# catniplab/vlgp

Hardware: AMD Instinct MI355X
Metric: EM iterations/sec (higher is better)
Workload: dtype f64

## Files before the change

vlgp_amd/csrc/ctx.h:

```cpp
#pragma once
#include <hip/hip_runtime.h>
#include <stdint.h>

#include <map>
#include <string>
#include <vector>

#include "../../include/vlgp_hip.h"

#define VLGP_WAVE 64
#define VLGP_E_LANES 4
#define VLGP_PRIOR_SLOTS 64

struct Prior {
    int T = 0;
    double* d_full = nullptr;
    double* d_compact = nullptr;
    std::vector<int> rl;
    std::vector<int64_t> goff;
    int64_t compact_len = 0;
    int index = -1;
};

enum : unsigned {
    SET_PLAIN = 1,
    SET_TILING = 2,
    SET_COPIED = 4,
    SET_GROUPS = 8,
    SET_MASKED = 16,
    SET_MASKED_FIT = 32,
    SET_REPLICATED = SET_GROUPS | SET_MASKED | SET_MASKED_FIT,
    SET_BY_ROW = SET_MASKED | SET_MASKED_FIT,
    SET_FIT = SET_PLAIN | SET_TILING | SET_COPIED | SET_MASKED_FIT,
    SET_SOURCE = 64,
    SET_ANY = 127,
};

struct Replicas {
    int src = -1;
    bool by_row = false, overlap = false;
    int n = 0, n_pairs = 0, nw = 0;
    int64_t rows_src = 0;
    int* d_ch = nullptr;
    int* d_pair = nullptr;
    unsigned long long* d_mask = nullptr;
    double* d_wconst = nullptr;
    double* d_nobs = nullptr;
    void* d_xa = nullptr;
    double xh[8] = {};
};

struct UnitSet {
    bool valid = false;
    int M = 0;
    int64_t rows = 0;
    int Tmax = 0, Tmin = 0;
    std::vector<int64_t> off;
    int64_t* d_off = nullptr;
    double *y = nullptr, *x = nullptr, *mu = nullptr, *v = nullptr, *w = nullptr, *dmu = nullptr;
    bool x_ones = true;
    bool alias = false;
    int parent = -1;
    std::vector<int64_t> src_start;
    int64_t* d_src_start = nullptr;
    int* d_unit_prior = nullptr;
    uint64_t prior_epoch = 0;
    double* d_xb = nullptr;
    double* d_mu_stash = nullptr;
    double* d_scratch = nullptr;
    int64_t scratch_len = 0;
    double rows_all_ranks = 0.0;
    std::vector<int> stage_start;
    std::vector<int> link_start;
    int* d_links = nullptr;
    int n_links = 0;
    bool share_mu = true;
    Replicas rep;
    int rep_users = 0;

    unsigned kind() const {
        if (rep.src >= 0) return !rep.by_row ? SET_GROUPS : (rep.n == 1 ? SET_MASKED_FIT : SET_MASKED);
        return alias ? SET_TILING : (parent >= 0 ? SET_COPIED : SET_PLAIN);
    }
    bool is(unsigned kinds) const { return (kind() & kinds) != 0; }
    bool is_source() const { return rep_users > 0; }
};

#define VLGP_SWITCHES(X)                                                                                                 \
    X("VLGP_ESTEP_SPLIT", estep_split, TRI, -1, 0, 1, "split E-step (chip-wide launches per phase): 0 never, 1 whatever the set's size") \
    X("VLGP_ESTEP_LSPLIT", estep_lsplit, TRI, -1, 0, 1, "long units (T > 64) on the split E-step: 0 never, 1 below 128 tasks too") \
    X("VLGP_ESTEP_GENERIC", estep_generic, FLAG, false, 0, 1, "E-step: the generic kernels only (a replicated set keeps the split E-step)") \
    X("VLGP_ESTEP_LANEPT", estep_lanept, TRI, -1, 0, 1, "split E-step: 0 keeps the wave-per-task kernels for ranks <= 14") \
    X("VLGP_ESTEP_NO_SHARED_G", estep_no_shared_g, FLAG, false, 0, 1, "split E-step: per-wave staging of G in the rank <= 16 launches, no lane-per-task launches") \
    X("VLGP_ESTEP_MIX", estep_mix, TRI, -1, 0, 1, "split E-step: 0 launches lane-per-task and wave-per-task latents separately") \
    X("VLGP_ESTEP_LANES", estep_lanes, INT, 0, 1, VLGP_E_LANES, "split E-step: number of stream lanes (default: by set size, one or two)") \
    X("VLGP_LANE_PRIO", lane_prio, INT, 0, 0, 3, "instruction priority of the lane-per-task launches' waves")                \
    X("VLGP_LANE_CLOCK", lane_clock, INT, 0, 0, 2, "phase clock of the lane-per-task launches: 1 factor, 2 mean (vlgp_debug_phase_clock)") \
    X("VLGP_MSTEP_GENERIC", mstep_generic, FLAG, false, 0, 1, "M-step: the loop-based kernels at any size")                    \
    X("VLGP_MSTEP_WG_PER_CU", mstep_wg_per_cu, REAL, 1.0, 0.0, 1e300, "M-step accumulation: workgroups per compute unit")       \
    X("VLGP_NOISE_PASSES", noise_passes, FLAG, false, 0, 1, "M-step: the noise variance by two passes over the rows, not from the moments") \
    X("VLGP_NO_MGRAPH", no_mgraph, FLAG, false, 0, 1, "M-step: enqueue every launch instead of replaying the captured graph") \
    X("VLGP_ICHOL_BLOCK", ichol_block, FLAG, false, 0, 1, "prior factor: lengths <= 64 through the workgroup kernel of the long ones") \
    X("VLGP_NORMS_BLOCKS", norms_blocks, INT, 256, 1, 1024, "norms pass: largest number of workgroups (its partial sums have 1024 slots)") \
    X("VLGP_HSTEP_DENSE", hstep_dense, FLAG, false, 0, 1, "H-step: the dense matrix-pipe round, never the low-rank one")     \
    X("VLGP_HSTEP_GENERIC", hstep_generic, FLAG, false, 0, 1, "H-step: the generic kernels (the reference's omega retry)")     \
    X("VLGP_HSTEP_LOWRANK", hstep_lowrank, FLAG, false, 0, 1, "H-step: the low-rank round whatever the size rule says")        \
    X("VLGP_HSTEP_GENERIC_SEG", hstep_generic_seg, FLAG, false, 0, 1, "H-step: windows 65 ... 128 on the generic kernels")     \
    X("VLGP_HSTEP_FUSE_TABLES", hstep_fuse_tables, FLAG, false, 0, 1, "H-step: every low-rank round workgroup factors its kernel blocks itself (rejected: slower)") \
    X("VLGP_HSTEP_NO_WLM", hstep_no_wlm, FLAG, false, 0, 1, "H-step: the rounds read w row-major, no latent-major copy")       \
    X("VLGP_HSTEP_LR_TOL", hstep_lr_tol, REAL, 1e-12, 0.0, 1e300, "H-step: relative tolerance of the low-rank round's rank prediction") \
    X("VLGP_DEBUG_OCC", debug_occ, FLAG, false, 0, 1, "print occupancy of the fast E-step launch and the H-step's fall-backs on stderr")
#define VLGP_SW_T_FLAG bool
#define VLGP_SW_T_TRI int
#define VLGP_SW_T_INT int
#define VLGP_SW_T_REAL double
struct Switches {
#define X(name, field, kind, def, lo, hi, what) VLGP_SW_T_##kind field = def;
    VLGP_SWITCHES(X)
#undef X
};
void vlgp_read_switches(struct vlgp_ctx* ctx);

struct ProfSlot {
    int64_t launches = 0;
    double ms = 0.0;
    double units = 0.0;
};

struct vlgp_ctx {
    int dev = 0;
    hipStream_t stream = nullptr;
    int N = 0, L = 0, P = 0, R = 0;
    int n_cu = 256;
    std::vector<uint8_t> gauss;
    int n_gauss = 0;
    int* d_gauss = nullptr;
    double *d_a = nullptr, *d_b = nullptr, *d_noise = nullptr, *d_da = nullptr, *d_db = nullptr;
    bool have_params = false;

    std::map<int, Prior> priors;
    uint64_t prior_epoch = 1;
    const double** d_prior_base = nullptr;
    int* d_prior_rl = nullptr;
    int64_t* d_prior_goff = nullptr;
    int prior_rows = 0;
    int* h_prior_mb = nullptr;
    int* d_prior_mb_host = nullptr;
    int* d_prior_mb = nullptr;
    unsigned long long prior_seq = 0;
    std::vector<struct Prior*> prior_pending;
    unsigned long long prior_pending_seq = 0;

    UnitSet sets[VLGP_MAX_SETS];

    hipStream_t mstream = nullptr;
    double* d_work_m = nullptr;
    int64_t work_m_len = 0;
    int* d_fail_m = nullptr;
    void* comm_m = nullptr;
    hipEvent_t ev_fork = nullptr, ev_m_start = nullptr, ev_m_done = nullptr;
    bool m_pending = false;
    void* m_graph_exec = nullptr;
    std::vector<double> m_graph_key;

    double* d_ecols = nullptr;
    int* d_fail = nullptr;
    unsigned long long* d_clk = nullptr;
    double* d_work = nullptr;
    int64_t work_len = 0;
    double* h_pinned = nullptr;
    int64_t pinned_len = 0;
    unsigned* d_hsync = nullptr;
    double* h_hres = nullptr;
    double* d_hres = nullptr;
    unsigned h_seq = 0;
    double* d_hmpart = nullptr;
    bool hprep = false;
    hipEvent_t ev_e_done = nullptr;
    bool e_done_valid = false;
    uint64_t hprep_epoch = 0, write_epoch = 0;
    double* d_hmom = nullptr;
    int64_t hmom_len = 0;
    const UnitSet* hmom_us = nullptr;
    int hmom_T = 0;
    bool hmom_bracket = false;
    double* d_hwlm = nullptr;
    int64_t hwlm_len = 0;
    bool hwlm_valid = false;
    struct LrThr { int T; double dt, tol; std::vector<double> om; };
    std::vector<LrThr> lr_thr;
    Switches sw;
    std::vector<const void*> lds_attr_done;
    int h_prio = 1;
    double last_h_ms = 0.0, last_m_ms = 0.0;
    double h_t0 = 0.0;
    int last_hstep_path = 0;
    double hstat[4] = {0.0, 0.0, 0.0, 0.0};

    bool prof_on = false;
    ProfSlot prof[VLGP_PROF_KINDS];
    hipEvent_t ev0 = nullptr, ev1 = nullptr;
    struct PendingProf { int kind; hipEvent_t a, b; double units; bool done; };
    std::vector<PendingProf> pending;

    void* comm = nullptr;
    void* shm = nullptr;
    void* shm_m = nullptr;
    void* hx = nullptr;
    int rank = 0, world = 1;

    hipStream_t elane[VLGP_E_LANES - 1] = {};
    hipEvent_t ev_e_fork = nullptr, ev_e_join[VLGP_E_LANES - 1] = {};
    int last_estep_path = 0;
    int lds_max = 64 * 1024;

    double* d_xwork = nullptr;
    double* h_xres = nullptr;
    double* d_xres = nullptr;
    unsigned long long x_seq = 0;
    int x_pending = 0;
    int x_set = -1;
    double* h_msnap = nullptr;
    double* d_msnap = nullptr;
    bool msnap_valid = false;
    double* h_stage_par = nullptr;
    double* h_stage_map = nullptr;
    double* d_stage_map = nullptr;
    hipEvent_t ev_stage_par = nullptr, ev_stage_map = nullptr;
    bool stage_par_busy = false, stage_map_busy = false;

    double* d_elbo = nullptr;
    int64_t elbo_len = 0;

    std::string err;
};

inline UnitSet& vlgp_rows_owner(vlgp_ctx* ctx, UnitSet& us) { return us.rep.src >= 0 ? ctx->sets[us.rep.src] : us; }

struct LoglikShape { int64_t slots, n_rate; int grid_y; const char* limit; };
inline LoglikShape vlgp_loglik_shape(const vlgp_ctx* ctx, const UnitSet& us) {
    if (us.is(SET_BY_ROW))
        return {(int64_t)us.rep.n * ctx->N, us.rep.rows_src * ctx->N, us.rep.n, "vlgp_loglik: at most 65535 replicas per masked set"};
    if (us.is(SET_GROUPS))
        return {us.rep.n_pairs, us.rep.rows_src * us.rep.n_pairs, us.rep.n_pairs,
                "vlgp_loglik: at most 65535 (replica, channel) pairs per set"};
    return {ctx->N, us.rows * ctx->N, 1, ""};
}

int vlgp_fail(vlgp_ctx* ctx, int code, const char* fmt, ...);
#define HIPCHK(ctx, call)                                                          \
    do {                                                                           \
        hipError_t e__ = (call);                                                   \
// ... 71 lines not shown
```

vlgp_amd/csrc/mstep.hip:

```cpp
#include <type_traits>

#include "ctx.h"
#include "fast_exp.h"

#ifndef M_TILE
#define M_TILE 256
#endif

enum { K_PREP = 0, K_NEWTON = 1, K_NOISE1 = 2, K_NOISE2 = 3 };
enum { K_MASKED = 4 };

struct MArgs {
    int N, L, P;
    int64_t rows;
    int rows_per_wg;
    int CT;
    int S;
    const double* y;
    const double* x;
    const double* mu;
    const double* v;
    const double* a;
    const double* b;
    union {
        const int* gauss;
        const unsigned long long* mask;
    };
    union {
        const double* mean;
        const double* nobs;
    };
    double* partial;
};

__host__ __device__ constexpr int tri(int n) { return n * (n + 1) / 2; }
template <int LT, int PT, int KINDM>
__host__ __device__ constexpr int nacc() {
    constexpr int KIND = KINDM & (K_MASKED - 1);
    return KIND == K_PREP ? LT + PT + PT * LT + tri(PT) + (PT <= 2 ? 2 + PT : 0)
         : KIND == K_NEWTON ? 2 * LT + tri(LT) + PT + tri(PT)
         : 1;
}
static inline int nstat_rt(int L, int P, int kind) {
    return kind == K_PREP ? L + P + P * L + tri(P) + (P <= 2 ? 2 + P : 0) : kind == K_NEWTON ? 2 * L + tri(L) + P + tri(P) : 1;
}

#define MS_GS 8
template <int LT, int PT, int KINDM, bool EXACT>
__global__ void __launch_bounds__(512, (LT <= 5 ? 4 : (LT <= 8 ? 2 : 1))) mstep_accum(MArgs A) {
    extern __shared__ __attribute__((aligned(16))) double smem[];
    constexpr int KIND = KINDM & (K_MASKED - 1);
    constexpr bool MASKED = (KINDM & K_MASKED) != 0;
    constexpr int NA = nacc<LT, PT, KIND>();
    constexpr int NBUF = 1;
    const int N = A.N, CT = A.CT, S = A.S;
    const int L = EXACT ? LT : A.L, P = EXACT ? PT : A.P;
    const int tid = threadIdx.x;
    const int nl = tid % CT, s = tid / CT;
    const int n = blockIdx.y * CT + nl;
    const bool active = s < S && n < N;
    const int tile_d = 2 * M_TILE * L;
    double* red = smem;
    const int red_d = MS_GS * S * CT;
    double* etab = smem + (NBUF * tile_d > red_d ? NBUF * tile_d : red_d);
    if constexpr (KIND == K_NEWTON) fast_exp_tab_init(etab, tid);

    double al[LT], al2[LT], bl[PT], acc[NA];
#pragma unroll
    for (int l = 0; l < LT; ++l) {
        al[l] = (active && l < L) ? A.a[l * N + n] : 0.0;
        al2[l] = 0.5 * al[l] * al[l];
    }
#pragma unroll
    for (int j = 0; j < PT; ++j) bl[j] = (active && j < P) ? A.b[j * N + n] : 0.0;
#pragma unroll
    for (int k = 0; k < NA; ++k) acc[k] = 0.0;
    const bool gch = (active && !MASKED) ? A.gauss[n] != 0 : false;
    const int nw = (N + 63) >> 6;
    if constexpr (MASKED && KIND == K_NEWTON) {
        if (active && s == 0 && blockIdx.x == 0 && A.nobs[n] == 0.0) {
#pragma unroll
            for (int i = 0; i < LT; ++i) acc[LT + tri(i) + i] = 1.0;
#pragma unroll
            for (int i = 0; i < PT; ++i) acc[2 * LT + tri(LT) + PT + tri(i) + i] = 1.0;
        }
    }
    const double shift = (KIND == K_NOISE2 && active) ? A.mean[n] : 0.0;

    const int64_t c0 = (int64_t)blockIdx.x * A.rows_per_wg;
    int64_t c1 = c0 + A.rows_per_wg;
    if (c1 > A.rows) c1 = A.rows;
    auto copy_tile = [&](double* buf, int64_t t0) {
        const int cnt = (int)((c1 - t0) < M_TILE ? (c1 - t0) : M_TILE) * L;
        for (int i = tid; i < cnt; i += blockDim.x) {
            buf[i] = A.mu[t0 * L + i];
            buf[M_TILE * L + i] = A.v[t0 * L + i];
        }
    };
    if (c0 < c1) copy_tile(smem, c0);
    __syncthreads();
    for (int64_t t0 = c0; t0 < c1; t0 += M_TILE) {
        const int nr = (int)((c1 - t0) < M_TILE ? (c1 - t0) : M_TILE);
        const bool more = t0 + M_TILE < c1;
        const double* mu_t = smem;
        const double* v_t = mu_t + M_TILE * L;
        if (active && !(KIND == K_NEWTON && gch)) {
#pragma unroll 2
        for (int rr = s; rr < nr; rr += S) {
            const int64_t row = t0 + rr;
            double xv[PT];
#pragma unroll
            for (int j = 0; j < PT; ++j)
                xv[j] = EXACT ? 1.0 : ((j < P) ? (A.x ? A.x[(row * P + j) * N + n] : 1.0) : 0.0);
            double mr[LT], vr[LT];
#pragma unroll
            for (int l = 0; l < LT; ++l) {
                mr[l] = (EXACT || l < L) ? mu_t[rr * L + l] : 0.0;
                vr[l] = (EXACT || l < L) ? v_t[rr * L + l] : 0.0;
            }
            auto observed = [&]() -> bool {
                return ((reinterpret_cast<const unsigned*>(A.mask)[row * (2 * nw) + (n >> 5)] >> (n & 31)) & 1u) == 0u;
            };
            if constexpr (KIND == K_PREP) {
                double yv = A.y[row * N + n];
                if constexpr (MASKED) yv = observed() ? yv : 0.0;
                int k = 0;
#pragma unroll
                for (int l = 0; l < LT; ++l) { acc[k] = fma(mr[l], yv, acc[k]); ++k; }
#pragma unroll
                for (int j = 0; j < PT; ++j) { acc[k] = fma(xv[j], yv, acc[k]); ++k; }
#pragma unroll
                for (int j = 0; j < PT; ++j)
#pragma unroll
                    for (int l = 0; l < LT; ++l) { acc[k] = fma(xv[j], mr[l], acc[k]); ++k; }
#pragma unroll
                for (int i = 0; i < PT; ++i)
#pragma unroll
                    for (int j = 0; j <= i; ++j) { acc[k] = fma(xv[i], xv[j], acc[k]); ++k; }
                if constexpr (PT <= 2) {
                    acc[k] = fma(yv, yv, acc[k]); ++k;
                    acc[k] += yv; ++k;
#pragma unroll
                    for (int j = 0; j < PT; ++j) { acc[k] += xv[j]; ++k; }
                }
            } else {
                double eta = 0.0;
#pragma unroll
                for (int j = 0; j < PT; ++j) eta = fma(xv[j], bl[j], eta);
#pragma unroll
                for (int l = 0; l < LT; ++l) eta = fma(mr[l], al[l], eta);
                if constexpr (KIND == K_NEWTON) {
                    double ex = eta;
#pragma unroll
                    for (int l = 0; l < LT; ++l) ex = fma(vr[l], al2[l], ex);
                    double rate = trunc_exp_tab64(ex, etab);
                    if constexpr (MASKED) rate = observed() ? rate : 0.0;
                    double mt[LT], q[LT];
#pragma unroll
                    for (int l = 0; l < LT; ++l) {
                        mt[l] = fma(vr[l], al[l], mr[l]);
                        q[l] = mt[l] * rate;
                    }
                    int k = 0;
#pragma unroll
                    for (int l = 0; l < LT; ++l) { acc[k] += q[l]; ++k; }
#pragma unroll
                    for (int i = 0; i < LT; ++i)
#pragma unroll
                        for (int j = 0; j <= i; ++j) { acc[k] = fma(q[i], mt[j], acc[k]); ++k; }
#pragma unroll
                    for (int l = 0; l < LT; ++l) { acc[k] = fma(rate, vr[l], acc[k]); ++k; }
#pragma unroll
                    for (int j = 0; j < PT; ++j) { acc[k] = fma(xv[j], rate, acc[k]); ++k; }
#pragma unroll
                    for (int i = 0; i < PT; ++i)
#pragma unroll
                        for (int j = 0; j <= i; ++j) { acc[k] = fma(xv[i] * xv[j], rate, acc[k]); ++k; }
                } else {
                    double dres = A.y[row * N + n] - eta - shift;
                    if constexpr (MASKED) dres = observed() ? dres : 0.0;
                    if constexpr (KIND == K_NOISE1) acc[0] += dres;
                    else acc[0] = fma(dres, dres, acc[0]);
                }
            }
        }
        }
        if (more) {
            __syncthreads();
            copy_tile(smem, t0 + M_TILE);
        }
        __syncthreads();
    }
    int kex[NA];
    {
        int k = 0, ke = 0;
        if constexpr (KIND == K_PREP) {
#pragma unroll
            for (int l = 0; l < LT; ++l, ++k) kex[k] = l < L ? ke++ : -1;
#pragma unroll
            for (int j = 0; j < PT; ++j, ++k) kex[k] = j < P ? ke++ : -1;
#pragma unroll
            for (int j = 0; j < PT; ++j)
#pragma unroll
                for (int l = 0; l < LT; ++l, ++k) kex[k] = (j < P && l < L) ? ke++ : -1;
#pragma unroll
            for (int i = 0; i < PT; ++i)
#pragma unroll
                for (int j = 0; j <= i; ++j, ++k) kex[k] = i < P ? ke++ : -1;
            if constexpr (PT <= 2) {
                kex[k++] = ke++;
                kex[k++] = ke++;
#pragma unroll
                for (int j = 0; j < PT; ++j, ++k) kex[k] = j < P ? ke++ : -1;
            }
        } else if constexpr (KIND == K_NEWTON) {
#pragma unroll
            for (int l = 0; l < LT; ++l, ++k) kex[k] = l < L ? ke++ : -1;
#pragma unroll
            for (int i = 0; i < LT; ++i)
#pragma unroll
                for (int j = 0; j <= i; ++j, ++k) kex[k] = i < L ? ke++ : -1;
#pragma unroll
            for (int l = 0; l < LT; ++l, ++k) kex[k] = l < L ? ke++ : -1;
#pragma unroll
            for (int j = 0; j < PT; ++j, ++k) kex[k] = j < P ? ke++ : -1;
#pragma unroll
            for (int i = 0; i < PT; ++i)
#pragma unroll
                for (int j = 0; j <= i; ++j, ++k) kex[k] = i < P ? ke++ : -1;
        } else {
            kex[0] = 0;
        }
    }
    const int K = KIND == K_PREP ? L + P + P * L + tri(P) + (P <= 2 ? 2 + P : 0) : KIND == K_NEWTON ? 2 * L + tri(L) + P + tri(P) : 1;
    const int SC = S * CT;
#pragma unroll
    for (int g0 = 0; g0 < NA; g0 += MS_GS) {
        if (s < S) {
#pragma unroll
            for (int j = 0; j < MS_GS; ++j)
                if (g0 + j < NA) red[j * SC + s * CT + nl] = active ? acc[g0 + j] : 0.0;
        }
        __syncthreads();
        for (int o = tid; o < MS_GS * CT; o += blockDim.x) {
            const int j = o / CT, c = o - j * CT;
            int ke = -1;
#pragma unroll
            for (int jj = 0; jj < MS_GS; ++jj)
                if (g0 + jj < NA && jj == j) ke = kex[g0 + jj];
            const int nn = blockIdx.y * CT + c;
            if (ke >= 0 && nn < N) {
                double t = 0.0;
                for (int q = 0; q < S; ++q) t += red[j * SC + q * CT + c];
                A.partial[((int64_t)blockIdx.x * K + ke) * N + nn] = t;
            }
        }
        if (g0 + MS_GS < NA) __syncthreads();
    }
}

__global__ void __launch_bounds__(512) sum_partials_kernel(const double* partial, int G, int64_t K, double* out) {
    __shared__ double red[8][64];
    const int o = threadIdx.x & 63, sl = threadIdx.x >> 6;
    const int64_t i = (int64_t)blockIdx.x * 64 + o;
    double s0 = 0.0, s1 = 0.0;
    if (i < K) {
        int g = sl;
        for (; g + 8 < G; g += 16) {
            s0 += partial[(int64_t)g * K + i];
            s1 += partial[(int64_t)(g + 8) * K + i];
        }
        if (g < G) s0 += partial[(int64_t)g * K + i];
    }
    red[sl][o] = s0 + s1;
    __syncthreads();
    if (sl == 0 && i < K) {
        double t = 0.0;
#pragma unroll
        for (int q = 0; q < 8; ++q) t += red[q][o];
        out[i] = t;
    }
}

template <int LT>
__global__ void __launch_bounds__(256)
latent_moments_kernel(int L, int64_t rows, const double* mu, const double* v, const double* dmu,
                      double* partial) {
    __shared__ double red[256];
    constexpr int NA = tri(LT) + 3 * LT + 1;
    double acc[NA];
#pragma unroll
    for (int k = 0; k < NA; ++k) acc[k] = 0.0;
    for (int64_t t = (int64_t)blockIdx.x * 256 + threadIdx.x; t < rows; t += (int64_t)gridDim.x * 256) {
        double mr[LT], vr[LT], dr[LT];
#pragma unroll
        for (int l = 0; l < LT; ++l) {
            mr[l] = l < L ? mu[t * L + l] : 0.0;
            vr[l] = (v && l < L) ? v[t * L + l] : 0.0;
            dr[l] = (dmu && l < L) ? dmu[t * L + l] : 0.0;
        }
        int k = 0;
#pragma unroll
        for (int i = 0; i < LT; ++i)
#pragma unroll
            for (int j = 0; j <= i; ++j) { acc[k] = fma(mr[i], mr[j], acc[k]); ++k; }
#pragma unroll
        for (int l = 0; l < LT; ++l) { acc[k] += mr[l]; ++k; }
#pragma unroll
        for (int l = 0; l < LT; ++l) { acc[k] += vr[l]; ++k; }
#pragma unroll
        for (int l = 0; l < LT; ++l) { acc[k] = fma(mr[l], mr[l], acc[k]); ++k; }
#pragma unroll
        for (int l = 0; l < LT; ++l) acc[k] = fma(dr[l], dr[l], acc[k]);
    }
    const int K = tri(L) + 3 * L + 1;
    auto emit = [&](int ke, double val) {
        __syncthreads();
        red[threadIdx.x] = val;
        __syncthreads();
        for (int o = 128; o > 0; o >>= 1) {
            if ((int)threadIdx.x < o) red[threadIdx.x] += red[threadIdx.x + o];
            __syncthreads();
        }
        if (threadIdx.x == 0) partial[(int64_t)blockIdx.x * K + ke] = red[0];
    };
    int k = 0, ke = 0;
#pragma unroll
    for (int i = 0; i < LT; ++i)
#pragma unroll
        for (int j = 0; j <= i; ++j, ++k) if (i < L) emit(ke++, acc[k]);
#pragma unroll
    for (int l = 0; l < LT; ++l, ++k) if (l < L) emit(ke++, acc[k]);
#pragma unroll
    for (int l = 0; l < LT; ++l, ++k) if (l < L) emit(ke++, acc[k]);
#pragma unroll
    for (int l = 0; l < LT; ++l, ++k) if (l < L) emit(ke++, acc[k]);
    emit(ke, acc[k]);
}


enum { T_ONE = 0, T_MU, T_V, T_MT, T_X, T_Y, T_C };
#define MG_CH 8

__device__ __forceinline__ void tri_ij(int k, int& i, int& j) {
// ... 563 lines not shown
            }
        }
        return;
    }
    if (kind == K_NEWTON && accum_exact(LT, PT, A.L, A.P, A.x == nullptr)) {
        hipLaunchKernelGGL((mstep_accum<LT, PT, K_NEWTON, true>), grid, blk, g.lds, st, A);
        return;
    }
    switch (kind) {
        case K_PREP: hipLaunchKernelGGL((mstep_accum<LT, PT, K_PREP, false>), grid, blk, g.lds, st, A); break;
        case K_NEWTON: hipLaunchKernelGGL((mstep_accum<LT, PT, K_NEWTON, false>), grid, blk, g.lds, st, A); break;
        case K_NOISE1: hipLaunchKernelGGL((mstep_accum<LT, PT, K_NOISE1, false>), grid, blk, g.lds, st, A); break;
        default: hipLaunchKernelGGL((mstep_accum<LT, PT, K_NOISE2, false>), grid, blk, g.lds, st, A); break;
    }
}
template <int LT>
static int launch_accum_p(vlgp_ctx* ctx, int kind, const Geometry& g, const MArgs& A) {
    hipStream_t mst = ctx->mstream;
    switch (accum_pt(A.P)) {
        case 1: launch_accum_k<LT, 1>(mst, kind, g, A); break;
        case 2: launch_accum_k<LT, 2>(mst, kind, g, A); break;
        case 4: launch_accum_k<LT, 4>(mst, kind, g, A); break;
        case 8: launch_accum_k<LT, 8>(mst, kind, g, A); break;
        default: return vlgp_fail(ctx, VLGP_ERR_ARG, "M-step kernel supports xdim <= 8, got %d", A.P);
    }
    HIPCHK(ctx, hipGetLastError());
    return VLGP_OK;
}
static bool mstep_generic(const vlgp_ctx* ctx, int L, int P) { return L > 16 || P > 8 || ctx->sw.mstep_generic; }
static int launch_accum_gen(vlgp_ctx* ctx, int kind, const Geometry& g, const MArgs& A, double* cache) {
    hipStream_t st = ctx->mstream;
    if (kind != K_PREP) {
        int64_t blocks = (A.rows * A.N + 255) / 256;
        if (blocks > 8192) blocks = 8192;
        hipLaunchKernelGGL(mstep_cache_gen, dim3((unsigned)blocks), dim3(256), 0, st, A, kind, cache);
    }
    const int K = nstat_rt(A.L, A.P, kind);
    hipLaunchKernelGGL(mstep_accum_gen, dim3(g.G, (A.N + 255) / 256, (K + MG_CH - 1) / MG_CH), dim3(256), 0, st, A, kind, K,
                       cache);
    HIPCHK(ctx, hipGetLastError());
    return VLGP_OK;
}

static int launch_accum(vlgp_ctx* ctx, int kind, const Geometry& g, const MArgs& A, double* cache = nullptr) {
    if (mstep_generic(ctx, A.L, A.P)) return launch_accum_gen(ctx, kind, g, A, cache);
    switch (accum_lt(A.L)) {
        case 2: return launch_accum_p<2>(ctx, kind, g, A);
        case 3: return launch_accum_p<3>(ctx, kind, g, A);
        case 5: return launch_accum_p<5>(ctx, kind, g, A);
        case 8: return launch_accum_p<8>(ctx, kind, g, A);
        case 10: return launch_accum_p<10>(ctx, kind, g, A);
        case 16: return launch_accum_p<16>(ctx, kind, g, A);
    }
    return vlgp_fail(ctx, VLGP_ERR_ARG, "M-step kernel supports at most 16 latents, got %d", A.L);
}

int mstep_plan_report(vlgp_ctx* ctx, int64_t rows, int out[12]) {
    const int L = ctx->L, P = ctx->P;
    const Geometry g = plan(ctx, rows);
    const bool gen = mstep_generic(ctx, L, P);
    const int lt = gen ? 0 : accum_lt(L), pt = gen ? 0 : accum_pt(P);
    const int fixed = solve_fixed(L, P);
    const int v[12] = {g.G, g.rows_per_wg, g.CT, g.S, g.nthr, g.tiles, lt, pt,
                       !gen && accum_exact(lt, pt, L, P, true), fixed, solve_anyg(ctx, fixed), noise_by_passes(ctx)};
    for (int i = 0; i < 12; ++i) out[i] = v[i];
    return VLGP_OK;
}

template <int LT>
static void launch_lat_t(hipStream_t st, int G, int L, int64_t rows, const double* mu, const double* v,
                         const double* dmu, double* partial) {
    hipLaunchKernelGGL((latent_moments_kernel<LT>), dim3(G), dim3(256), 0, st, L, rows, mu, v, dmu, partial);
}

static int latent_moments_st(vlgp_ctx* ctx, UnitSet& us, double* d_partial, double* d_out, hipStream_t st) {
    const int L = ctx->L;
    int G = (int)((us.rows + 255) / 256);
    if (G > 256) G = 256;
    if (G < 1) G = 1;
    const int K = tri(L) + 3 * L + 1;
    if (L > 16 || ctx->sw.mstep_generic)
        hipLaunchKernelGGL(latent_moments_gen, dim3(G, (K + MG_CH - 1) / MG_CH), dim3(256), 0, st, L, us.rows, us.mu, us.v,
                           us.dmu, d_partial);
    else if (L <= 2) launch_lat_t<2>(st, G, L, us.rows, us.mu, us.v, us.dmu, d_partial);
    else if (L <= 3) launch_lat_t<3>(st, G, L, us.rows, us.mu, us.v, us.dmu, d_partial);
    else if (L <= 5) launch_lat_t<5>(st, G, L, us.rows, us.mu, us.v, us.dmu, d_partial);
    else if (L <= 8) launch_lat_t<8>(st, G, L, us.rows, us.mu, us.v, us.dmu, d_partial);
    else if (L <= 10) launch_lat_t<10>(st, G, L, us.rows, us.mu, us.v, us.dmu, d_partial);
    else launch_lat_t<16>(st, G, L, us.rows, us.mu, us.v, us.dmu, d_partial);
    HIPCHK(ctx, hipGetLastError());
    hipLaunchKernelGGL(sum_partials_kernel, dim3((K + 63) / 64), dim3(512), 0, st, d_partial, G,
                       (int64_t)K, d_out);
    HIPCHK(ctx, hipGetLastError());
    return VLGP_OK;
}
static int latent_moments(vlgp_ctx* ctx, UnitSet& us, double* d_partial, double* d_out, bool mlane) {
    CHK(latent_moments_st(ctx, us, d_partial, d_out, mlane ? ctx->mstream : ctx->stream));
    const int K = tri(ctx->L) + 3 * ctx->L + 1;
    return mlane ? vlgp_allreduce_m(ctx, d_out, K) : vlgp_allreduce(ctx, d_out, K);
}

int launch_moments(vlgp_ctx* ctx, UnitSet& us) {
    const int L = ctx->L;
    const int K = tri(L) + 3 * L + 1;
    CHK(vlgp_ensure_work(ctx, 256LL * K + K + 64));
    double* d_partial = ctx->d_work + K + 64;
    return latent_moments(ctx, us, d_partial, ctx->d_work, false);
}

int launch_mstep(vlgp_ctx* ctx, UnitSet& us, int n_iter, int use_hessian, double eps, double lr,
                 double da_bound, double db_bound) {
    const int N = ctx->N, L = ctx->L, P = ctx->P;
    const bool gen = mstep_generic(ctx, L, P);
    const bool masked = us.is(SET_REPLICATED);
    if (masked) {
        if (ctx->n_gauss > 0)
            return vlgp_fail(ctx, VLGP_ERR_STATE, "masked M-step: the handle has Gaussian channels (their least-squares "
                             "update needs per-channel masked Gram matrices)");
        if (gen)
            return vlgp_fail(ctx, VLGP_ERR_STATE, "masked M-step: the loop-based M-step kernels (P > 8 or "
                             "VLGP_MSTEP_GENERIC) take no mask");
        if (L > 10) return vlgp_fail(ctx, VLGP_ERR_STATE, "masked M-step: more than 10 latents (L > 10)");
        if (ctx->world > 1) return vlgp_fail(ctx, VLGP_ERR_STATE, "masked M-step: more than one rank");
        if (!us.is(SET_MASKED_FIT) || !us.rep.d_mask || !us.rep.d_nobs) return vlgp_fail(ctx, VLGP_ERR_STATE, "masked M-step: the set has no mask");
    }
    const int km = masked ? K_MASKED : 0;
    const Geometry g = plan(ctx, us.rows);
    const int Kp = nstat_rt(L, P, K_PREP), Kn = nstat_rt(L, P, K_NEWTON);
    const int Kl = tri(L) + 3 * L + 1;
    const int Kmax = Kp > Kn ? Kp : Kn;
    const int64_t o_prep = 0, o_stats = o_prep + (int64_t)Kp * N, o_lat = o_stats + (int64_t)Kn * N;
    const int64_t o_s1 = o_lat + Kl + 8, o_mean = o_s1 + N, o_tick = o_mean + N, o_part = o_tick + 2;
    int64_t part_len = (int64_t)g.G * Kmax * N;
    if (part_len < 256LL * Kl) part_len = 256LL * Kl;
    const int Dg = L > P ? L : P;
    const int64_t o_cache = o_part + part_len, o_hws = o_cache + (gen ? us.rows * N : 0);
    CHK(vlgp_ensure_work_m(ctx, o_hws + (gen ? (int64_t)N * Dg * (Dg + 3) : 0)));
    double* W = ctx->d_work_m;
    hipStream_t st = ctx->mstream;
    double *d_prep = W + o_prep, *d_stats = W + o_stats, *d_lat = W + o_lat, *d_s1 = W + o_s1,
           *d_mean = W + o_mean, *d_part = W + o_part;
    double* d_cache = gen ? W + o_cache : nullptr;
    unsigned* d_ticket = reinterpret_cast<unsigned*>(W + o_tick);

    const bool use_graph = ctx->world == 1 && !ctx->prof_on && !ctx->sw.no_mgraph;
    const bool noise_passes = masked || noise_by_passes(ctx);
    std::vector<double> key;
    if (use_graph) {
        auto pk = [&](const void* p_) { key.push_back((double)(uintptr_t)p_); };
        pk(us.y); pk(us.x_ones ? nullptr : us.x); pk(us.mu); pk(us.v); pk(us.w); pk(us.dmu); pk(W); pk(ctx->d_a); pk(ctx->d_b);
        pk(ctx->d_noise); pk(ctx->d_da); pk(ctx->d_db); pk(ctx->d_fail_m); pk(ctx->d_gauss);
        pk(masked ? us.rep.d_mask : nullptr); pk(masked ? us.rep.d_nobs : nullptr); key.push_back((double)masked);
        for (double v_ : {(double)us.rows, (double)N, (double)L, (double)P, (double)ctx->n_gauss, (double)n_iter,
                          (double)use_hessian, eps, lr, da_bound, db_bound, (double)noise_passes, (double)gen, ctx->sw.mstep_wg_per_cu})
            key.push_back(v_);
        if (ctx->m_graph_exec && key == ctx->m_graph_key) {
            HIPCHK(ctx, hipGraphLaunch(static_cast<hipGraphExec_t>(ctx->m_graph_exec), st));
            return VLGP_OK;
        }
        if (ctx->m_graph_exec) {
            (void)hipGraphExecDestroy(static_cast<hipGraphExec_t>(ctx->m_graph_exec));
            ctx->m_graph_exec = nullptr;
        }
        HIPCHK(ctx, hipStreamBeginCapture(st, hipStreamCaptureModeThreadLocal));
    }
    auto enqueue = [&]() -> int {
    HIPCHK(ctx, hipMemsetAsync(d_ticket, 0, sizeof(double) * 2, st));

    MArgs A;
    A.N = N; A.L = L; A.P = P; A.rows = us.rows; A.rows_per_wg = g.rows_per_wg; A.CT = g.CT; A.S = g.S;
    A.y = us.y; A.x = us.x_ones ? nullptr : us.x; A.mu = us.mu; A.v = us.v;
    A.a = ctx->d_a; A.b = ctx->d_b; A.gauss = ctx->d_gauss; A.mean = d_mean; A.partial = d_part;
    if (masked) A.mask = us.rep.d_mask;

    auto reduce_to = [&](int K, double* dst) -> int {
        const int64_t n = (int64_t)K * N;
        hipLaunchKernelGGL(sum_partials_kernel, dim3((unsigned)((n + 63) / 64)), dim3(512), 0, st,
                           d_part, g.G, n, dst);
        HIPCHK(ctx, hipGetLastError());
        return vlgp_allreduce_m(ctx, dst, n);
    };

    CHK(launch_accum(ctx, K_PREP | km, g, A, d_cache));
    CHK(reduce_to(Kp, d_prep));
    CHK(latent_moments(ctx, us, d_part, d_lat, true));
    double total_rows = (double)us.rows;
    if (ctx->world > 1 && us.rows_all_ranks > 0.0) {
        total_rows = us.rows_all_ranks;
    } else if (ctx->world > 1) {
        double h = total_rows;
        HIPCHK(ctx, hipMemcpyAsync(d_lat + Kl, &h, sizeof(double), hipMemcpyHostToDevice, st));
        HIPCHK(ctx, hipStreamSynchronize(st));
        CHK(vlgp_allreduce_m(ctx, d_lat + Kl, 1));
        HIPCHK(ctx, hipMemcpyAsync(&h, d_lat + Kl, sizeof(double), hipMemcpyDeviceToHost, st));
        HIPCHK(ctx, hipStreamSynchronize(st));
        total_rows = h;
        us.rows_all_ranks = h;
    }

    SolveArgs S;
    S.N = N; S.L = L; S.P = P; S.use_hessian = use_hessian; S.eps = eps; S.lr = lr;
    S.da_bound = da_bound; S.db_bound = db_bound;
    S.prep = d_prep; S.stats = d_stats; S.lat = d_lat; S.gauss = ctx->d_gauss;
    S.a = ctx->d_a; S.b = ctx->d_b; S.da = ctx->d_da; S.db = ctx->d_db; S.fail = ctx->d_fail_m;
    S.hws = gen ? W + o_hws : nullptr;

    const bool any_poisson = ctx->n_gauss < N;
    for (int it = 0; it < n_iter; ++it) {
        if (it == n_iter - 1) {
            if (!noise_passes) {
                hipLaunchKernelGGL(noise_stats_kernel, dim3((N + 255) / 256), dim3(256), 0, st, N, L, P, total_rows,
                                   d_prep, d_lat, ctx->d_a, ctx->d_b, ctx->d_noise);
                HIPCHK(ctx, hipGetLastError());
            } else {
            CHK(launch_accum(ctx, K_NOISE1 | km, g, A, d_cache));
            CHK(reduce_to(1, d_s1));
            if (masked) hipLaunchKernelGGL(noise_mean_nobs_kernel, dim3((N + 255) / 256), dim3(256), 0, st, N, us.rep.d_nobs, d_s1, d_mean);
            else hipLaunchKernelGGL(noise_mean_kernel, dim3((N + 255) / 256), dim3(256), 0, st, N,
                               total_rows, d_s1, d_mean);
            CHK(launch_accum(ctx, K_NOISE2 | km, g, A, d_cache));
            CHK(reduce_to(1, d_s1));
            if (masked) hipLaunchKernelGGL(noise_final_nobs_kernel, dim3((N + 255) / 256), dim3(256), 0, st, N, us.rep.d_nobs, d_s1, ctx->d_noise);
            else hipLaunchKernelGGL(noise_final_kernel, dim3((N + 255) / 256), dim3(256), 0, st, N,
                               total_rows, d_s1, ctx->d_noise);
            HIPCHK(ctx, hipGetLastError());
            }
        }
        if (any_poisson) {
            vlgp_prof_begin(ctx, VLGP_PROF_MSTEP, st);
            MArgs An = A;
            if (masked) An.nobs = us.rep.d_nobs;
            int rc = launch_accum(ctx, K_NEWTON | km, g, An, d_cache);
            vlgp_prof_end(ctx, VLGP_PROF_MSTEP, (double)us.rows, st);
            CHK(rc);
            if (ctx->world == 1) {
                const int64_t n = (int64_t)Kn * N;
                const dim3 sg((unsigned)((n + MS_OUT - 1) / MS_OUT));
                const int fixed = solve_fixed(L, P);
                const bool anyg = solve_anyg(ctx, fixed);
#define MS_SUM_SOLVE(F)                                                                                                  \
    do {                                                                                                                  \
        if (anyg) hipLaunchKernelGGL((mstep_sum_solve_kernel<F, true>), sg, dim3(512), 0, st, d_part, g.G, n, d_stats, d_ticket, S);  \
        else hipLaunchKernelGGL((mstep_sum_solve_kernel<F, false>), sg, dim3(512), 0, st, d_part, g.G, n, d_stats, d_ticket, S);      \
    } while (0)
                if (fixed == 3) MS_SUM_SOLVE(3);
                else if (fixed == 5) MS_SUM_SOLVE(5);
                else if (fixed == 8) MS_SUM_SOLVE(8);
                else if (fixed == 10) MS_SUM_SOLVE(10);
#undef MS_SUM_SOLVE
                else hipLaunchKernelGGL(mstep_sum_solve_kernel<0>, sg, dim3(512), 0, st, d_part, g.G, n, d_stats, d_ticket, S);
                HIPCHK(ctx, hipGetLastError());
                continue;
            }
            CHK(reduce_to(Kn, d_stats));
        }
        hipLaunchKernelGGL(mstep_solve_kernel, dim3((N + 63) / 64), dim3(64), 0, st, S);
        HIPCHK(ctx, hipGetLastError());
    }
    return VLGP_OK;
    };
    const int rc = enqueue();
    if (!use_graph) return rc;
    hipGraph_t graph = nullptr;
    const hipError_t ec = hipStreamEndCapture(st, &graph);
    if (rc != VLGP_OK) {
        if (graph) (void)hipGraphDestroy(graph);
        return rc;
    }
    HIPCHK(ctx, ec);
    hipGraphExec_t exec = nullptr;
    const hipError_t ei = hipGraphInstantiate(&exec, graph, nullptr, nullptr, 0);
    (void)hipGraphDestroy(graph);
    HIPCHK(ctx, ei);
    ctx->m_graph_exec = exec;
    ctx->m_graph_key = key;
    HIPCHK(ctx, hipGraphLaunch(exec, st));
    return VLGP_OK;
}
```

Baseline: 154.4.

## Double-buffer M-step row tiles with direct-to-LDS async loads

The M-step accumulation kernel now stages mu and v in half tiles with two alternating LDS buffers. The next half is prefetched through global_load_lds direct-to-LDS loads while the current half is consumed, replacing the load-then-sync-then-compute copy. LDS reads go through pointers that advance by row stride. The kernel also aliases the x*x accumulator to the x accumulator when P is 1, dropping redundant FMAs. A switch keeps the old synchronous staging, and the change adds alignment-dependent code paths and rides on a hardware intrinsic.

After: 153.0. About the same (-0.9%).

```diff
diff --git a/vlgp_amd/csrc/ctx.h b/vlgp_amd/csrc/ctx.h
--- a/vlgp_amd/csrc/ctx.h
+++ b/vlgp_amd/csrc/ctx.h
@@ -98,6 +98,7 @@
     X("VLGP_LANE_CLOCK", lane_clock, INT, 0, 0, 2, "phase clock of the lane-per-task launches: 1 factor, 2 mean (vlgp_debug_phase_clock)") \
     X("VLGP_MSTEP_GENERIC", mstep_generic, FLAG, false, 0, 1, "M-step: the loop-based kernels at any size")                    \
     X("VLGP_MSTEP_WG_PER_CU", mstep_wg_per_cu, REAL, 1.0, 0.0, 1e300, "M-step accumulation: workgroups per compute unit")       \
+    X("VLGP_MSTEP_SYNC_STAGE", mstep_sync_stage, FLAG, false, 0, 1, "M-step accumulation: stage every row tile by plain loads + LDS stores, no direct-to-LDS loads") \
     X("VLGP_NOISE_PASSES", noise_passes, FLAG, false, 0, 1, "M-step: the noise variance by two passes over the rows, not from the moments") \
     X("VLGP_NO_MGRAPH", no_mgraph, FLAG, false, 0, 1, "M-step: enqueue every launch instead of replaying the captured graph") \
     X("VLGP_ICHOL_BLOCK", ichol_block, FLAG, false, 0, 1, "prior factor: lengths <= 64 through the workgroup kernel of the long ones") \
diff --git a/vlgp_amd/csrc/mstep.hip b/vlgp_amd/csrc/mstep.hip
--- a/vlgp_amd/csrc/mstep.hip
+++ b/vlgp_amd/csrc/mstep.hip
@@ -6,6 +6,9 @@
 #ifndef M_TILE
 #define M_TILE 256
 #endif
+#define M_HALF (M_TILE / 2)
+#define MS_GLOBAL __attribute__((address_space(1)))
+#define MS_LDS __attribute__((address_space(3)))
 
 enum { K_PREP = 0, K_NEWTON = 1, K_NOISE1 = 2, K_NOISE2 = 3 };
 enum { K_MASKED = 4 };
@@ -16,6 +19,7 @@
     int rows_per_wg;
     int CT;
     int S;
+    int sync_stage;
     const double* y;
     const double* x;
     const double* mu;
@@ -53,6 +57,7 @@
     constexpr bool MASKED = (KINDM & K_MASKED) != 0;
     constexpr int NA = nacc<LT, PT, KIND>();
     constexpr int NBUF = 1;
+    constexpr bool ALIAS_XX = EXACT && KIND == K_NEWTON && PT == 1;
     const int N = A.N, CT = A.CT, S = A.S;
     const int L = EXACT ? LT : A.L, P = EXACT ? PT : A.P;
     const int tid = threadIdx.x;
@@ -77,12 +82,16 @@
     for (int k = 0; k < NA; ++k) acc[k] = 0.0;
     const bool gch = (active && !MASKED) ? A.gauss[n] != 0 : false;
     const int nw = (N + 63) >> 6;
+    bool no_obs = false;
     if constexpr (MASKED && KIND == K_NEWTON) {
-        if (active && s == 0 && blockIdx.x == 0 && A.nobs[n] == 0.0) {
+        no_obs = active && s == 0 && blockIdx.x == 0 && A.nobs[n] == 0.0;
+        if (no_obs) {
 #pragma unroll
             for (int i = 0; i < LT; ++i) acc[LT + tri(i) + i] = 1.0;
-#pragma unroll
-            for (int i = 0; i < PT; ++i) acc[2 * LT + tri(LT) + PT + tri(i) + i] = 1.0;
+            if constexpr (!ALIAS_XX) {
+#pragma unroll
+                for (int i = 0; i < PT; ++i) acc[2 * LT + tri(LT) + PT + tri(i) + i] = 1.0;
+            }
         }
     }
     const double shift = (KIND == K_NOISE2 && active) ? A.mean[n] : 0.0;
@@ -90,24 +99,43 @@
     const int64_t c0 = (int64_t)blockIdx.x * A.rows_per_wg;
     int64_t c1 = c0 + A.rows_per_wg;
     if (c1 > A.rows) c1 = A.rows;
-    auto copy_tile = [&](double* buf, int64_t t0) {
-        const int cnt = (int)((c1 - t0) < M_TILE ? (c1 - t0) : M_TILE) * L;
-        for (int i = tid; i < cnt; i += blockDim.x) {
-            buf[i] = A.mu[t0 * L + i];
-            buf[M_TILE * L + i] = A.v[t0 * L + i];
+    const int hl = M_HALF * L;
+    const int lane = tid & 63;
+    const int wfirst = __builtin_amdgcn_readfirstlane(tid - lane);
+    auto stage_half = [&](double* buf, int64_t h0) {
+        const int cnt = (int)((c1 - h0) < M_HALF ? (c1 - h0) : M_HALF) * L;
+        const double* gm = A.mu + h0 * L;
+        const double* gv = A.v + h0 * L;
+        const bool direct = !A.sync_stage && ((reinterpret_cast<uintptr_t>(gm) | reinterpret_cast<uintptr_t>(gv)) & 15) == 0;
+        const int np = direct ? cnt >> 1 : 0;
+        for (int p = wfirst; p < np; p += (int)blockDim.x) {
+            if (p + lane < np) {
+                __builtin_amdgcn_global_load_lds((const MS_GLOBAL double*)gm + 2 * (p + lane),
+                                                 (MS_LDS double*)buf + 2 * p, 16, 0, 0);
+                __builtin_amdgcn_global_load_lds((const MS_GLOBAL double*)gv + 2 * (p + lane),
+                                                 (MS_LDS double*)buf + hl + 2 * p, 16, 0, 0);
+            }
+        }
+        for (int i = 2 * np + tid; i < cnt; i += (int)blockDim.x) {
+            buf[i] = gm[i];
+            buf[hl + i] = gv[i];
         }
     };
-    if (c0 < c1) copy_tile(smem, c0);
+    if (c0 < c1) stage_half(smem, c0);
     __syncthreads();
-    for (int64_t t0 = c0; t0 < c1; t0 += M_TILE) {
-        const int nr = (int)((c1 - t0) < M_TILE ? (c1 - t0) : M_TILE);
-        const bool more = t0 + M_TILE < c1;
-        const double* mu_t = smem;
-        const double* v_t = mu_t + M_TILE * L;
+    int hb = 0, rr = s;
+    for (int64_t h0 = c0; h0 < c1; h0 += M_HALF, hb ^= 1) {
+        const int nh = (int)((c1 - h0) < M_HALF ? (c1 - h0) : M_HALF);
+        double* half = smem + hb * 2 * hl;
+        if (h0 + M_HALF < c1) stage_half(smem + (hb ^ 1) * 2 * hl, h0 + M_HALF);
         if (active && !(KIND == K_NEWTON && gch)) {
+        const MS_LDS double* mp = (const MS_LDS double*)half + rr * L;
+        const MS_LDS double* vp = mp + hl;
+        asm volatile("" : "+v"(vp));
+        const int rstep = S * L;
 #pragma unroll 2
-        for (int rr = s; rr < nr; rr += S) {
-            const int64_t row = t0 + rr;
+        for (; rr < nh; rr += S, mp += rstep, vp += rstep) {
+            const int64_t row = h0 + rr;
             double xv[PT];
 #pragma unroll
             for (int j = 0; j < PT; ++j)
@@ -115,8 +143,8 @@
             double mr[LT], vr[LT];
 #pragma unroll
             for (int l = 0; l < LT; ++l) {
-                mr[l] = (EXACT || l < L) ? mu_t[rr * L + l] : 0.0;
-                vr[l] = (EXACT || l < L) ? v_t[rr * L + l] : 0.0;
+                mr[l] = (EXACT || l < L) ? mp[l] : 0.0;
+                vr[l] = (EXACT || l < L) ? vp[l] : 0.0;
             }
             auto observed = [&]() -> bool {
                 return ((reinterpret_cast<const unsigned*>(A.mask)[row * (2 * nw) + (n >> 5)] >> (n & 31)) & 1u) == 0u;
@@ -172,10 +200,12 @@
                     for (int l = 0; l < LT; ++l) { acc[k] = fma(rate, vr[l], acc[k]); ++k; }
 #pragma unroll
                     for (int j = 0; j < PT; ++j) { acc[k] = fma(xv[j], rate, acc[k]); ++k; }
-#pragma unroll
-                    for (int i = 0; i < PT; ++i)
-#pragma unroll
-                        for (int j = 0; j <= i; ++j) { acc[k] = fma(xv[i] * xv[j], rate, acc[k]); ++k; }
+                    if constexpr (!ALIAS_XX) {
+#pragma unroll
+                        for (int i = 0; i < PT; ++i)
+#pragma unroll
+                            for (int j = 0; j <= i; ++j) { acc[k] = fma(xv[i] * xv[j], rate, acc[k]); ++k; }
+                    }
                 } else {
                     double dres = A.y[row * N + n] - eta - shift;
                     if constexpr (MASKED) dres = observed() ? dres : 0.0;
@@ -185,11 +215,13 @@
             }
         }
         }
-        if (more) {
-            __syncthreads();
-            copy_tile(smem, t0 + M_TILE);
-        }
+        rr = hb ? s : rr - M_HALF;
         __syncthreads();
+    }
+    if constexpr (ALIAS_XX) {
+        constexpr int kx = 2 * LT + tri(LT);
+        acc[kx + 1] = acc[kx];
+        if (no_obs) acc[kx + 1] = 1.0 + acc[kx];
     }
     int kex[NA];
     {
@@ -1059,7 +1091,8 @@
         pk(ctx->d_noise); pk(ctx->d_da); pk(ctx->d_db); pk(ctx->d_fail_m); pk(ctx->d_gauss);
         pk(masked ? us.rep.d_mask : nullptr); pk(masked ? us.rep.d_nobs : nullptr); key.push_back((double)masked);
         for (double v_ : {(double)us.rows, (double)N, (double)L, (double)P, (double)ctx->n_gauss, (double)n_iter,
-                          (double)use_hessian, eps, lr, da_bound, db_bound, (double)noise_passes, (double)gen, ctx->sw.mstep_wg_per_cu})
+                          (double)use_hessian, eps, lr, da_bound, db_bound, (double)noise_passes, (double)gen, ctx->sw.mstep_wg_per_cu,
+                          (double)ctx->sw.mstep_sync_stage})
             key.push_back(v_);
         if (ctx->m_graph_exec && key == ctx->m_graph_key) {
             HIPCHK(ctx, hipGraphLaunch(static_cast<hipGraphExec_t>(ctx->m_graph_exec), st));
@@ -1076,6 +1109,7 @@
 
     MArgs A;
     A.N = N; A.L = L; A.P = P; A.rows = us.rows; A.rows_per_wg = g.rows_per_wg; A.CT = g.CT; A.S = g.S;
+    A.sync_stage = ctx->sw.mstep_sync_stage;
     A.y = us.y; A.x = us.x_ones ? nullptr : us.x; A.mu = us.mu; A.v = us.v;
     A.a = ctx->d_a; A.b = ctx->d_b; A.gauss = ctx->d_gauss; A.mean = d_mean; A.partial = d_part;
     if (masked) A.mask = us.rep.d_mask;
```
